# ctu-mrs/space_filling_forest_star

Measured on AMD Instinct MI355X. Metric: accepted node expansions/sec + collision checks/sec, dense_3D 6-DoF, higher is better.
Workload: dtype f64

## Files before the change

### space_filling_forest_star_amd/csrc/commit_next.h

```cpp
#pragma once
#include <stdint.h>
#include "kernels.h"
#include "sff_pmath.h"

namespace sffk {

struct CommitRegs {
  int32_t n_act, halt, n_nodes, iter, round, solved, fault, N0, iter0, n_borders, frontier_n, act_sel, act_cnt;
  int32_t app_n, app_N0, app_fn0, app_act_sel, iter0_app, app_act_cnt, app_nb0;
  unsigned long long cursor, words_base, rounds, round_nodes, round_queries, epoch;
};

SFF_HD CommitRegs commit_regs_load(const DevCtrl* c, int32_t nb0) {
  CommitRegs k{};
  k.n_act = c->n_act; k.halt = c->halt; k.iter = c->iter; k.round = c->round; k.solved = c->solved;
  k.N0 = c->N0; k.iter0 = c->iter0; k.n_borders = nb0; k.frontier_n = c->frontier_n;
  k.act_sel = c->act_sel; k.act_cnt = c->act_cnt; k.cursor = c->cursor; k.epoch = c->epoch;
  return k;
}

template <class C> SFF_HD void round_begin_next(const DevForestView& f, C* c) {
  const int cnt = c->act_cnt;
  int n = 0;
  if (c->round < f.threshold_misses && cnt > 0 && c->iter < f.max_iterations && !c->solved) {
// ... 42 lines not shown
  if (faulted) { commit_roll_back(k); return; }
  k->app_n = k->n_act;
  k->app_N0 = k->N0;
  k->app_fn0 = k->frontier_n;
  k->app_act_sel = k->act_sel;
  k->app_act_cnt = k->act_cnt;
  k->iter0_app = k->iter0;
  k->app_nb0 = k->n_borders;
  k->epoch += 1ULL;
}

template <class C> SFF_HD void commit_next_round(const DevForestView& f, C* k, int n_acc, int n_ev, bool faulted) {
  commit_applied(k, faulted);
  if (faulted) return;
  const int n = k->app_n, fn0 = k->app_fn0, act_cnt = k->app_act_cnt;
  k->n_nodes = k->app_N0 + n_acc;
  k->frontier_n = f.prio.n_heaps ? fn0 : fn0 + n_acc;
  k->n_borders = k->app_nb0 + n_ev;
  k->act_sel = k->app_act_sel ^ 1;
  k->act_cnt = (n - n_acc) + (act_cnt - n);
  round_begin_next(f, k);
}

}
```

### space_filling_forest_star_amd/csrc/devforest.hip

```cpp
#include <hip/hip_runtime.h>
#include <stdint.h>
#include <stdlib.h>
#include "kernels.h"
#include "sff_geom.h"
#include "kernels_dev.h"
#include "commit_next.h"

namespace sffk {

using namespace sffg;

__device__ __forceinline__ int record_words_dev(int nbcap) { return 6 + 4 * nbcap; }

__device__ __forceinline__ int32_t* frontier_now(const DevForestView& f) { return f.ctrl->front_sel ? f.frontier2 : f.frontier; }
__device__ __forceinline__ int32_t* act_now(const DevForestView& f) { return f.ctrl->act_sel ? f.act_slot2 : f.act_slot; }

__device__ void round_begin_scalars(const DevForestView& f, DevCtrl* c) { round_begin_next(f, c); }

#define WB_BLOCKS 64
__global__ __launch_bounds__(256) void k_wave_begin(DevForestView f) {
  __shared__ int s_last;
  __shared__ int s_scan[4];
  DevCtrl* c = f.ctrl;
  const unsigned long long tb0 = f.profile ? wall_clock64() : 0ULL;
// ... 165 lines not shown
  __syncthreads();
  if (threadIdx.x < 8) slots[threadIdx.x] = 0ULL;
  __syncthreads();
  if ((threadIdx.x & 63) == 0)
    for (int q = from; q < 8; ++q) if (v[q]) atomicAdd(&slots[q], v[q]);
  __syncthreads();
  for (int q = from; q < 8; ++q) v[q] = slots[q];
}

__device__ __forceinline__ void commit_counters(DevCtrl& K, const unsigned long long* tot, int work_items, bool have_q,
                                                unsigned long long q_beg, unsigned long long q_end) {
  K.collide_calls += tot[0];
  K.path_free_calls += tot[1];
  K.nn_queries += tot[2];
  K.poses_executed += tot[3];
  K.segments_executed += tot[4];
  K.samples_executed += tot[5];
  K.n_unsettled += (int)tot[6];
  K.work_items += (unsigned long long)work_items;
  if (have_q) { K.q_t0 = q_beg; K.q_t1 = q_end; }
  if (K.q_t1 > K.q_t0) { K.q_ticks += K.q_t1 - K.q_t0; K.q_launches += 1ULL; }
}

__global__ __launch_bounds__(1024) void k_commit(ResolveArgs A, int n_bound) {
  __shared__ int s_state[64], s_dk[64], s_dep[64];
  __shared__ unsigned long long s_cnt[64][6];
  __shared__ unsigned long long s_sum;
  __shared__ unsigned long long s_wa, s_we, s_c6[7];
  __shared__ int s_ev_total;
  __shared__ unsigned long long s_tot[8];
  __shared__ DevCtrl K;
  const DevForestView& f = A.f;
  DevCtrl* c = f.ctrl;
  const int b = blockIdx.x;
  const int grp = threadIdx.x >> 4, gl = threadIdx.x & 15, lane = threadIdx.x & 63;
  const int i = b * 64 + grp;
  const bool inb = i < n_bound;
  const size_t s0 = (size_t)i * A.stride;
  const bool inl = inb && A.in_lim[i] != 0;
  const int flags = inb ? A.rec_flags[i] : 0;
  int nnb = inb ? A.rec_nnb[i] : 0;
  const bool pose_hit = inb && A.pose_hit[i] != 0;
  int fh = 0x7fffffff, ns = 0, nb = 0, meta = 0;
  if (inb) {
    fh = A.first_hit[s0 + gl]; ns = A.seg_ns[s0 + gl];
    if (gl > 0) { nb = A.rec_nb[(size_t)i * A.nbcap + gl - 1]; meta = A.rec_meta[(size_t)i * A.nbcap + gl - 1]; }
  }
  const int halt = c->halt, n = c->n_act;
  if (halt || n == 0) {
    if (b == 0 && threadIdx.x == 0) {
      c->app_n = 0;
      if (A.star) { A.S.hdr[0] = 0; A.S.hdr[1] = 1; A.S.hdr[2] = 0; A.S.hdr[4] = 0; }
    }
    return;
  }
  if (b == 0 && f.ord.hist)
    for (int r = threadIdx.x; r < f.ord.n_sub; r += 1024) (c->act_sel ? f.ord.cnt[0] : f.ord.cnt[1])[r * SFFK_ORD_CNT_STRIDE] = 0;
  if (b * 64 >= n) return;
  const int nwg = (n + 63) >> 6;
  const bool last = b == nwg - 1;
  const unsigned seq = (unsigned)f.commit_seq[0] + 1u;
  const int seq30 = (int)(seq & 0x3fffffffu);
  const int Tb = f.temp_base, N0 = c->N0, nb0 = c->n_borders;
  const unsigned long long stamp_hi = (c->epoch + 1ULL) << 32;
  unsigned long long* pub = f.wg_pub + (size_t)b * SFFK_PUB_WORDS;
  unsigned long long tk[6];
  const bool clk = last && f.profile;
  tk[0] = clk ? wall_clock64() : 0ULL;
  unsigned long long* trace = (f.kc_trace && (int)c->rounds == f.kc_trace_round && threadIdx.x == 0) ? f.kc_trace + 8 * (size_t)b : nullptr;
#define KC_TRACE(k) do { if (trace) trace[k] = wall_clock64(); } while (0)
  KC_TRACE(0);
  const bool tail = last && A.star;
  int work_items = 0;
  if (tail) {
    for (int w = threadIdx.x; w < (int)(sizeof(DevCtrl) / 4); w += 1024)
      reinterpret_cast<int32_t*>(&K)[w] = reinterpret_cast<const int32_t*>(c)[w];
    work_items = A.round_ctrl[2];
  }
  if (!A.star && b == 0 && threadIdx.x < 64) {
    unsigned long long q_end = f.qclk_sh[threadIdx.x * 16], q_beg = f.qclk_sh[threadIdx.x * 16 + 1];
    const int wi = A.round_ctrl[2];
    for (int off = 32; off > 0; off >>= 1) {
      const unsigned long long e2 = __shfl_xor(q_end, off), b2 = __shfl_xor(q_beg, off);
      q_end = e2 > q_end ? e2 : q_end; q_beg = b2 < q_beg ? b2 : q_beg;
    }
    if (threadIdx.x == 0) {
      f.qclk_sh[KH_QBEG] = q_beg; f.qclk_sh[KH_QEND] = q_end; f.qclk_sh[KH_WORK] = (unsigned long long)wi;
      f.qclk_sh[KH_NB0] = (unsigned long long)(unsigned)nb0;
    }
  }

  auto calls_of = [](int fh, int ns) -> unsigned long long {
    return fh != 0x7fffffff ? (unsigned long long)fh : (unsigned long long)ns;
  };
  const int gsh = lane & 48;
  auto gballot = [&](bool p) -> unsigned { return (unsigned)((__ballot(p) >> gsh) & 0xffffULL); };
  auto gsum = [&](unsigned long long v) -> unsigned long long {
    for (int off = 8; off > 0; off >>= 1) v += __shfl_xor(v, off);
    return v;
  };
  unsigned long long cnt[6] = {0, 0, 0, 0, 0, 0};
  int st = 1, code = SFFK_REJECTED, dk = 0, was_dep = 0;
// ... 118 lines not shown
    const unsigned long long wa = __ballot(v == 2), we = __ballot(v == 3), wd = __ballot(s_dep[threadIdx.x] != 0);
    unsigned long long c6[6];
    for (int q = 0; q < 6; ++q) {
      c6[q] = s_cnt[threadIdx.x][q];
      for (int off = 32; off > 0; off >>= 1) c6[q] += __shfl_xor(c6[q], off);
    }
    if (threadIdx.x == 0) {
      s_wa = wa; s_we = we;
      for (int q = 0; q < 6; ++q) s_c6[q] = c6[q];
      s_c6[6] = (unsigned long long)__popcll(wd);
      f.w_acc[b] = wa;
      for (int q = 0; q < 6; ++q) kc_publish(pub + KC_CNT + q, seq, (unsigned)c6[q]);
      kc_publish(pub + KC_DEP, seq, (unsigned)__popcll(wd));
      kc_publish(pub + KC_EVN, seq, (unsigned)__popcll(we));
      kc_publish(pub + KC_WLO, seq, (unsigned)(wa & 0xffffffffULL));
      kc_publish(pub + KC_WHI, seq, (unsigned)(wa >> 32));
      kc_publish(pub + KC_ACC, seq, (unsigned)__popcll(wa));
      KC_TRACE(2);
      f.w_ev[b] = we;
    }
  }
  __syncthreads();
  const unsigned long long wa = s_wa, we = s_we;
  const bool defer = !A.star;
  int e_nb = 0, e_ex = 0, e_i = 0;
  size_t e_h = 0;
  bool is_ev = false, stamped = false, posted = false;
  if (threadIdx.x < 64) {
    if ((we >> threadIdx.x) & 1ULL) {
      is_ev = true;
      e_i = b * 64 + (int)threadIdx.x;
      const int raw = A.rec_nb[(size_t)e_i * A.nbcap + s_dk[threadIdx.x]];
      e_ex = A.parent[e_i];
      if (raw < Tb) {
        e_nb = raw;
        const int a = e_nb < e_ex ? e_nb : e_ex, bb = e_nb < e_ex ? e_ex : e_nb;
        const unsigned long long key = ((unsigned long long)(uint32_t)a << 32) | ((unsigned long long)(uint32_t)bb + 1ULL);
        e_h = border_slot(f, key);
        atomicMin(&f.bt_val[e_h], stamp_hi | (unsigned long long)(uint32_t)e_i);
        stamped = true;
        if (defer) { f.ev_h[e_i] = (unsigned long long)e_h; f.ev_nb[e_i] = e_nb; f.ev_raw[e_i] = raw; }
      }
    }
    if (!defer && __ballot(is_ev && !stamped) == 0ULL) {
      if (we != 0ULL) __threadfence();
      if (threadIdx.x == 0) {
        kc_publish(pub + KC_POSTED, seq, 1u);
        if (we == 0ULL) kc_publish(pub + KC_OWN, seq, 0u);
      }
      posted = true;
    }
  }
  unsigned long long part = 0;
  if ((int)threadIdx.x < b) part = kc_wait(f.wg_pub + (size_t)threadIdx.x * SFFK_PUB_WORDS + KC_ACC, seq, f.commit_seq + 6);
  unsigned long long early[8] = {0, 0, 0, 0, 0, 0, 0, 0};
  if (tail && (int)threadIdx.x < b)
    for (int q = 0; q < 8; ++q) early[q] = kc_load(f.wg_pub + (size_t)threadIdx.x * SFFK_PUB_WORDS + KC_CNT + q);
  const int acc_pref = (int)kc_block_sum(part, &s_sum);
  int fault_seen = 0;
  if (tail && threadIdx.x == 1023) fault_seen = __hip_atomic_load(A.fault_pending, __ATOMIC_RELAXED, __HIP_MEMORY_SCOPE_AGENT);
  if (threadIdx.x == 0) {
    f.acc_pref[b] = acc_pref;
    kc_publish(pub + KC_PREF, seq, (unsigned)acc_pref);
  }
  if (A.star && threadIdx.x < 64 && ((wa >> threadIdx.x) & 1ULL))
    A.S.acc_sample[acc_pref + __popcll(wa & ((1ULL << threadIdx.x) - 1ULL))] = b * 64 + (int)threadIdx.x;
  if (clk) tk[2] = wall_clock64();
  KC_TRACE(4);
  int n_own = 0, ev_pref = 0;
  if (f.profile && !A.star && threadIdx.x < 64) {
    const unsigned long long wm = __ballot(is_ev && !stamped);
    if (threadIdx.x == 0 && wm) atomicAdd(&f.qclk_sh[KH_MATE_EV], (unsigned long long)__popcll(wm));
  }
  if (we != 0ULL || last) {
    if (is_ev && !stamped) {
      const int raw = A.rec_nb[(size_t)e_i * A.nbcap + s_dk[threadIdx.x]];
      const int j = raw - Tb, bj = j >> 6;
      int pj = acc_pref;
      unsigned long long wj = wa;
      if (bj != b) {
        const unsigned long long* pp = f.wg_pub + (size_t)bj * SFFK_PUB_WORDS;
        pj = (int)kc_wait(pp + KC_PREF, seq, f.commit_seq + 6);
        wj = (unsigned long long)kc_wait(pp + KC_WLO, seq, f.commit_seq + 6) |
             ((unsigned long long)kc_wait(pp + KC_WHI, seq, f.commit_seq + 6) << 32);
      }
      e_nb = N0 + pj + __popcll(wj & ((1ULL << (j & 63)) - 1ULL));
      const int a = e_nb < e_ex ? e_nb : e_ex, bb = e_nb < e_ex ? e_ex : e_nb;
      const unsigned long long key = ((unsigned long long)(uint32_t)a << 32) | ((unsigned long long)(uint32_t)bb + 1ULL);
      e_h = border_slot(f, key);
      atomicMin(&f.bt_val[e_h], stamp_hi | (unsigned long long)(uint32_t)e_i);
      if (defer) { f.ev_h[e_i] = (unsigned long long)e_h; f.ev_nb[e_i] = e_nb; f.ev_raw[e_i] = raw; }
    }
  }
  if (!defer && (we != 0ULL || last)) {
    if (threadIdx.x < 64 && !posted) {
      if (we != 0ULL) __threadfence();
      if (threadIdx.x == 0) kc_publish(pub + KC_POSTED, seq, 1u);
    }
    KC_TRACE(3);
    if (we != 0ULL && (int)threadIdx.x < b) (void)kc_wait(f.wg_pub + (size_t)threadIdx.x * SFFK_PUB_WORDS + KC_POSTED, seq, f.commit_seq + 6);
    __syncthreads();
    KC_TRACE(5);
    bool own = false;
    if (is_ev) {
      const unsigned long long owner = __hip_atomic_load(&f.bt_val[e_h], __ATOMIC_RELAXED, __HIP_MEMORY_SCOPE_AGENT);
// ... 11 lines not shown
      if ((int)threadIdx.x < b) pe = kc_wait(f.wg_pub + (size_t)threadIdx.x * SFFK_PUB_WORDS + KC_OWN, seq, f.commit_seq + 6);
      ev_pref = (int)kc_block_sum(pe, &s_sum);
    }
    KC_TRACE(6);
    if (own) {
      const int at = nb0 + ev_pref + __popcll(wo & ((1ULL << threadIdx.x) - 1ULL));
      double pn[6], pe6[6], dn;
      int ta;
      const int raw = A.rec_nb[(size_t)e_i * A.nbcap + s_dk[threadIdx.x]];
      if (raw >= Tb) {
        const int j = raw - Tb;
        for (int q = 0; q < 6; ++q) pn[q] = A.newpos[6 * (size_t)j + q];
        dn = A.pdist[j] + f.d_root[A.parent[j]];
        ta = A.st.tree[A.parent[j]];
      } else {
        for (int q = 0; q < 6; ++q) pn[q] = A.st.pos[6 * (size_t)e_nb + q];
        dn = f.d_root[e_nb];
        ta = A.st.tree[e_nb];
      }
      const int tb = A.st.tree[e_ex];
      f.b_n1[at] = e_nb < e_ex ? e_nb : e_ex; f.b_n2[at] = e_nb < e_ex ? e_ex : e_nb;
      f.b_ta[at] = ta < tb ? ta : tb; f.b_tb[at] = ta < tb ? tb : ta;
      for (int q = 0; q < 6; ++q) pe6[q] = A.st.pos[6 * (size_t)e_ex + q];
      if (A.star) {
        const int e = at - nb0;
        A.S.ev_sample[e] = e_i; A.S.ev_nb[e] = e_nb; A.S.ev_ex[e] = e_ex; A.S.ev_dist[e] = dist6(pn, pe6);
        f.b_dist[at] = 0.0;
      } else
      f.b_dist[at] = dn + f.d_root[e_ex] + dist6(pn, pe6);
      f.pair[(size_t)ta * f.n_trees + tb] = 1;
      f.pair[(size_t)tb * f.n_trees + ta] = 1;
    }
  }
  KC_TRACE(7);
  if (last && !A.star && threadIdx.x == 0) {
    f.qclk_sh[KH_PASSES] = (unsigned long long)passes;
    if (clk) {
      tk[3] = wall_clock64();
      for (int q = 0; q < 3; ++q) f.qclk_sh[KH_PHASE + q] = tk[q + 1] - tk[q];
    }
  }
  if (!tail) return;
  if (clk) tk[3] = wall_clock64();
  unsigned long long q_end = 0ULL, q_beg = ~0ULL;
  if (f.qclk_sh && threadIdx.x < 64) {
    q_end = f.qclk_sh[threadIdx.x * 16]; q_beg = f.qclk_sh[threadIdx.x * 16 + 1];
    for (int off = 32; off > 0; off >>= 1) {
      const unsigned long long e2 = __shfl_xor(q_end, off), b2 = __shfl_xor(q_beg, off);
      q_end = e2 > q_end ? e2 : q_end; q_beg = b2 < q_beg ? b2 : q_beg;
    }
  }
  unsigned long long tot[8] = {0, 0, 0, 0, 0, 0, 0, 0};
  if ((int)threadIdx.x < b) {
    const unsigned long long* pp = f.wg_pub + (size_t)threadIdx.x * SFFK_PUB_WORDS;
    for (int q = 0; q < 8; ++q) tot[q] = (unsigned)(early[q] >> 32) == seq ? (unsigned)early[q] : kc_wait(pp + KC_CNT + q, seq, f.commit_seq + 6);
  }
  if (threadIdx.x == 1023) s_ev_total = fault_seen;
  kc_block_sum8(tot, s_tot, 0);
  for (int q = 0; q < 7; ++q) tot[q] += s_c6[q];
  tot[7] += (unsigned long long)__popcll(we);
  const int n_acc = acc_pref + __popcll(wa), n_ev = defer ? (int)tot[7] : ev_pref + n_own;
  const bool faulted = s_ev_total != 0;
  if (A.star && !faulted) {
    for (int w = threadIdx.x; w < (int)(sizeof(DevCtrl) / 4); w += 1024)
      reinterpret_cast<int32_t*>(A.S.backup)[w] = reinterpret_cast<const int32_t*>(&K)[w];
    __syncthreads();
    if (threadIdx.x == 0) commit_roll_back(A.S.backup);
  }
  if (threadIdx.x == 0) {
    if (faulted) {
      commit_roll_back(&K);
      *A.fault_pending = 0;
      if (A.star) { A.S.hdr[0] = 0; A.S.hdr[1] = 1; A.S.hdr[2] = 0; A.S.hdr[4] = 0; }
    } else {
      commit_counters(K, tot, work_items, f.qclk_sh != nullptr, q_beg, q_end);
      commit_next_round(f, &K, n_acc, n_ev, false);
      if (A.star) {
        K.nn_queries += (unsigned long long)n_acc;
        A.S.hdr[0] = n_acc; A.S.hdr[1] = 0; A.S.hdr[2] = n_ev; A.S.hdr[3] = nb0; A.S.hdr[4] = 0;
      }
      if (clk) {
        tk[4] = wall_clock64();
        for (int q = 0; q < 4; ++q) K.prof[q] += tk[q + 1] - tk[q];
      }
      K.prof[5] += (unsigned long long)passes;
      K.prof[6] += 1ULL;
      if ((unsigned long long)passes > K.prof[7]) K.prof[7] = (unsigned long long)passes;
    }
    f.commit_seq[0] = (int32_t)seq;
  }
  __syncthreads();
  for (int w = threadIdx.x; w < (int)(sizeof(DevCtrl) / 4); w += 1024)
    reinterpret_cast<int32_t*>(c)[w] = reinterpret_cast<const int32_t*>(&K)[w];
}

struct AppCtl {
  int32_t n, N0, fn0, act_sel, act_cnt, iter0, nb0;
  int32_t new_cnt;
  int32_t wave_over;
  int32_t ord_valid;
// ... 30 lines not shown
  h.fault = A.fault_pending[0];
  h.seq0 = f.commit_seq[0];
  return h;
}
__device__ __forceinline__ void hand_join(HandIn& h) {
  join_v(h.k.n_act, h.k.halt, h.k.iter, h.k.round, h.k.solved, h.k.N0, h.k.iter0, h.k.n_borders, h.k.frontier_n, h.k.act_sel,
         h.k.act_cnt, h.k.cursor, h.k.epoch, h.in_wave, h.use_closed, h.ord_valid, h.n_slots, h.act_identity, h.fault, h.seq0,
         h.acc, h.evn);
}
__device__ __forceinline__ bool hand_ran(const HandIn& h) { return !(h.k.halt || h.k.n_act == 0); }
__device__ __forceinline__ void hand_count_in(const ResolveArgs& A) {
  atomicAdd(&A.f.qclk_sh[(blockIdx.x & 63) * 16 + KH_READY], 1ULL);
}
__device__ __forceinline__ AppCtl hand_app_ctl(const HandIn& h, const CommitRegs& k) {
  AppCtl a{};
  a.n = k.app_n; a.N0 = k.app_N0; a.fn0 = k.app_fn0; a.act_sel = k.app_act_sel; a.act_cnt = k.app_act_cnt;
  a.iter0 = k.iter0_app; a.nb0 = k.app_nb0; a.new_cnt = k.act_cnt;
  a.wave_over = (k.n_act == 0 && !k.halt && h.in_wave && !h.use_closed) ? 1 : 0;
  a.ord_valid = h.ord_valid;
  a.seq = (unsigned)h.seq0 + 1u;
  a.epoch = k.epoch;
  return a;
}
__device__ __forceinline__ AppCtl hand_applied(const ResolveArgs& A, const HandIn& h) {
  if (!hand_ran(h)) { AppCtl a{}; a.ord_valid = h.ord_valid; return a; }
  __syncthreads();
  if (threadIdx.x == 0) hand_count_in(A);
  CommitRegs k = h.k;
  commit_applied(&k, h.fault != 0);
  return hand_app_ctl(h, k);
}
__device__ __forceinline__ AppCtl hand_derive(const ResolveArgs& A, HandIn& h, int n_lines, unsigned long long* s_part) {
  const DevForestView& f = A.f;
  if (!hand_ran(h)) { AppCtl a{}; a.ord_valid = h.ord_valid; return a; }
  const unsigned seq = (unsigned)h.seq0 + 1u;
  auto line = [&](unsigned long long acc, unsigned long long evn) -> unsigned long long {
    return ((unsigned)(acc >> 32) == seq ? (unsigned long long)(unsigned)acc : 0ULL) |
           ((unsigned)(evn >> 32) == seq ? (unsigned long long)(unsigned)evn << 32 : 0ULL);
  };
  unsigned long long v = (int)threadIdx.x < n_lines ? line(h.acc, h.evn) : 0ULL;
  for (int t = threadIdx.x + 256; t < n_lines; t += 256) {
    const unsigned long long* pp = f.wg_pub + (size_t)t * SFFK_PUB_WORDS;
    v += line(pp[KC_ACC], pp[KC_EVN]);
  }
  unsigned pk = (unsigned)v | ((unsigned)(v >> 32) << 16);
  for (int off = 32; off > 0; off >>= 1) pk += __shfl_xor(pk, off);
  if ((threadIdx.x & 63) == 0) s_part[threadIdx.x >> 6] = (unsigned long long)(pk & 0xffffu) | ((unsigned long long)(pk >> 16) << 32);
  __syncthreads();
  if (threadIdx.x == 0) hand_count_in(A);
  v = s_part[0] + s_part[1] + s_part[2] + s_part[3];
  commit_next_round(f, &h.k, (int)(unsigned)v, (int)(v >> 32), h.fault != 0);
  return hand_app_ctl(h, h.k);
}
__device__ __forceinline__ void append_ord_store(const ResolveArgs& A, const AppCtl& C, int ord_at, int next) {
  if (ord_at >= 0) (C.act_sel ? A.f.ord.lst[0] : A.f.ord.lst[1])[ord_at] = next;
}
__device__ __forceinline__ int append_one(const ResolveArgs& A, const AppCtl& C, int i, int& slot_out, int& ord_at, int part = 0) {
  ord_at = -1;
  const DevForestView& f = A.f;
  const int n = C.n;
  slot_out = -1;
  if (n <= 0) return -1;
  const int act_cnt = C.act_cnt;
  const int32_t* act_old = C.act_sel ? f.act_slot2 : f.act_slot;
  int32_t* act_new = C.act_sel ? f.act_slot : f.act_slot2;
  const bool wave_over = C.wave_over != 0;
  const bool ord_on = f.ord.hist && C.ord_valid;
  auto claim = [&](int e, int slot) {
    const int nd = f.slot_node[slot];
    atomicMin(&f.claim[nd], e);
    f.ulist[e] = nd;
  };
  if (wave_over && i == 0 && part != 1) f.ctrl->claims_done = 1;
  if (i >= n) {
    if (i < act_cnt && part != 1) {
      const int e = (C.new_cnt - (act_cnt - n)) + (i - n), slot = act_old[i];
      act_new[e] = slot;
      if (wave_over) claim(e, slot);
    }
    return -1;
  }
  const unsigned long long w = f.w_acc[i >> 6];
  const int rank = f.acc_pref[i >> 6] + __popcll(w & ((1ULL << (i & 63)) - 1ULL));
  if (!((w >> (i & 63)) & 1ULL)) {
    auto ord_append = [&](int slot) {
      const int sub = f.ord.slot_pos[slot] >> 6;
      const bool first = C.act_sel != 0;
      ord_at = sub * 64 + atomicAdd(&(first ? f.ord.cnt[0] : f.ord.cnt[1])[sub * SFFK_ORD_CNT_STRIDE], 1);
    };
    if (part == 1) {
      if (ord_on) { ord_append(act_old[i]); append_ord_store(A, C, ord_at, i - rank); }
      return -1;
    }
    slot_out = act_old[i];
    act_new[i - rank] = slot_out;
    if (ord_on && part == 0) ord_append(slot_out);
    if (wave_over) claim(i - rank, slot_out);
    return i - rank;
  }
  if (A.star) return -1;
  const int N0 = C.N0, fn0 = C.fn0;
  int32_t* const frontier = frontier_now(f);
  const int id = N0 + rank;
  const int ex = A.parent[i];
  const double* p = A.newpos + 6 * (size_t)i;
  const size_t o = (size_t)id;
// ... 142 lines not shown
    if (!faulted) {
      if (f.profile) {
        for (int q = 0; q < 3; ++q) K.prof[q] += s_stash[KH_PHASE - KH_QBEG + q];
        K.prof[3] += wall_clock64() - t0;
        K.prof[4] += s_stash[KH_MATE_EV - KH_QBEG];
      }
      K.prof[5] += passes;
      K.prof[6] += 1ULL;
      if (passes > K.prof[7]) K.prof[7] = passes;
    } else {
      *A.fault_pending = 0;
    }
    f.commit_seq[0] = (int32_t)seq;
  }
  __syncthreads();
  constexpr int W_NB = (int)(offsetof(DevCtrl, n_borders) / 4), W_CD = (int)(offsetof(DevCtrl, claims_done) / 4),
                W_Q0 = (int)(offsetof(DevCtrl, q_t0) / 4), W_Q1 = (int)(offsetof(DevCtrl, q_ticks) / 4);
  for (int w = tid; w < (int)(sizeof(DevCtrl) / 4); w += 256) {
    if (w == W_NB || w == W_CD || (sampler && w >= W_Q0 && w < W_Q1)) continue;
    reinterpret_cast<int32_t*>(c)[w] = reinterpret_cast<const int32_t*>(&K)[w];
  }
}
__global__ __launch_bounds__(256) void k_append(ResolveArgs A, int append_blocks, int n_lines) {
  __shared__ unsigned long long s_hand[4];
  if (!A.star && blockIdx.x == gridDim.x - 1) { commit_finalize(A, (int)gridDim.x - 1, false); return; }
  const bool border = (int)blockIdx.x >= append_blocks;
  AppCtl C;
  if (A.star) C = app_ctl_block(A.f);
  else if (border) {
    HandIn h = hand_request<false>(A, n_lines);
    hand_join(h);
    C = hand_applied(A, h);
  } else {
    HandIn h = hand_request<true>(A, n_lines);
    hand_join(h);
    C = hand_derive(A, h, n_lines, s_hand);
  }
  if (border) { border_finalize(A, C, (int)blockIdx.x - append_blocks); return; }
  int slot, ord_at;
  const int next = append_one(A, C, blockIdx.x * 256 + threadIdx.x, slot, ord_at);
  append_ord_store(A, C, ord_at, next);
}
struct ListOne { int i, n, act_cnt, app_sel, new_cnt, slot, ex, next; bool wave_over; };
__device__ __forceinline__ void append_list_request(const ResolveArgs& A, int i, int bound, int n_lines, HandIn& h, SampleCtl& K,
                                                    ListOne& L) {
  const DevForestView& f = A.f;
  const DevCtrl* c = f.ctrl;
  const int ic = i < bound ? i : bound - 1;
  if (!A.star) h = hand_request<true>(A, n_lines);
  unsigned long long w = f.w_acc[ic >> 6];
  int pref = f.acc_pref[ic >> 6];
  int s0 = f.act_slot[ic], s1 = f.act_slot2[ic];
  int ex = A.parent[ic];
  L.i = i; L.n = 0; L.act_cnt = 0; L.app_sel = 0; L.new_cnt = 0; L.wave_over = false;
  if (A.star) {
    K = sample_ctl(c);
    int n = c->app_n, act_cnt = c->app_act_cnt, app_sel = c->app_act_sel, new_cnt = c->act_cnt;
    int in_wave = c->in_wave, use_closed = c->use_closed;
    join_ctl_v(K);
    join_v(n, act_cnt, app_sel, new_cnt, in_wave, use_closed, w, pref, s0, s1, ex);
    L.n = n; L.act_cnt = act_cnt; L.app_sel = app_sel; L.new_cnt = new_cnt;
    L.wave_over = K.n == 0 && !K.halt && in_wave && !use_closed;
  } else {
    hand_join(h);
    join_v(w, pref, s0, s1, ex);
    K = SampleCtl{};
    K.words_base = h.k.cursor;
    if (hand_ran(h)) {
      CommitRegs k = h.k;
      commit_applied(&k, h.fault != 0);
      L.n = k.app_n; L.act_cnt = k.app_act_cnt; L.app_sel = k.app_act_sel;
    }
  }
  L.slot = L.app_sel ? s1 : s0;
  L.ex = ex;
  L.next = (i < L.n && !((w >> (i & 63)) & 1ULL)) ? i - (pref + __popcll(w & ((1ULL << (i & 63)) - 1ULL))) : -1;
}
__device__ __forceinline__ void append_list_store(const ResolveArgs& A, const ListOne& L) {
  const DevForestView& f = A.f;
  const int i = L.i, n = L.n;
  if (n <= 0) return;
  int32_t* act_new = L.app_sel ? f.act_slot : f.act_slot2;
  if (L.wave_over && i == 0) f.ctrl->claims_done = 1;
  if (i >= n) {
    if (i < L.act_cnt) {
      const int e = (L.new_cnt - (L.act_cnt - n)) + (i - n);
      act_new[e] = L.slot;
      if (L.wave_over) { const int nd = f.slot_node[L.slot]; atomicMin(&f.claim[nd], e); f.ulist[e] = nd; }
    }
    return;
  }
  if (L.next < 0) return;
  act_new[L.next] = L.slot;
  if (L.wave_over) { atomicMin(&f.claim[L.ex], L.next); f.ulist[L.next] = L.ex; }
}
__global__ __launch_bounds__(256) void k_append_sample(ResolveArgs A, SampleLaunch P, int append_blocks, int n_lines) {
  __shared__ unsigned long long s_hand[4];
  if (!A.star && blockIdx.x == gridDim.x - 1) { commit_finalize(A, (int)gridDim.x - 1, true); return; }
  const int nb = append_blocks;
  const bool sampler = (int)blockIdx.x >= nb && (int)blockIdx.x < 2 * nb;
  if (!sampler) {
    AppCtl C;
    if (A.star) C = app_ctl_block(A.f);
    else {
      HandIn h = hand_request<false>(A, n_lines);
      hand_join(h);
      C = hand_applied(A, h);
    }
    if ((int)blockIdx.x >= 2 * nb) { border_finalize(A, C, (int)blockIdx.x - 2 * nb); return; }
    int slot, ord_at;
    (void)append_one(A, C, blockIdx.x * 256 + threadIdx.x, slot, ord_at, 1);
    return;
  }
  const int tid = ((int)blockIdx.x - nb) * 256 + threadIdx.x;
  HandIn h{};
  SampleCtl K;
  ListOne L;
  append_list_request(A, tid, P.n, n_lines, h, K, L);
  if (!A.star) {
    const AppCtl C = hand_derive(A, h, n_lines, s_hand);
    K.n = h.k.n_act; K.halt = h.k.halt; K.act_sel = h.k.act_sel; K.round = h.k.round;
    K.ord_valid = h.ord_valid; K.n_slots = h.n_slots; K.act_identity = h.act_identity;
    L.new_cnt = C.new_cnt; L.wave_over = C.wave_over != 0;
  }
  append_list_store(A, L);
  if (K.halt) return;
  const bool valid = L.next >= 0 && L.next < K.n;
  const SampleIn S = sample_fetch(valid ? L.next : 0, valid ? L.ex : 0, K, P);
  sample_finish(tid, valid, L.next, valid ? L.ex : 0, S, -1, K, P);
}

__device__ void wave_end_control(const DevForestView& f, DevCtrl* c, int removed, int fn, bool from_closed, int n_fail,
                                 const int32_t* grid_ovf, const int32_t* tgrid_ovf, const unsigned long long* star_s) {
  c->closed_n += removed;
  if (f.prio.n_heaps) {
    c->compact_from = 0;
    c->empty_frontier = c->prio_all_empty;
  } else {
    c->compact_from = removed > 0 ? fn : 0;
    c->frontier_n = fn - removed;
    if (removed > 0) c->front_sel ^= 1;
    c->empty_frontier = c->frontier_n == 0 ? 1 : 0;
  }
  if (!c->solved && c->empty_frontier && f.goal_id < 0) {
    const int R = f.n_trees;
    int reached = 1;
    for (int t = 0; t < R; ++t) f.claim[t] = t == 0 ? 1 : 0;
// ... 219 lines not shown
  else if (k < 4 + 2 * A.nbcap) A.rec_meta[(size_t)i * A.nbcap + (k - 4 - A.nbcap)] = v;
  else if (k < 4 + 2 * A.nbcap + A.stride) A.seg_ns[s0 + (k - 4 - 2 * A.nbcap)] = v;
  else A.first_hit[s0 + (k - 4 - 2 * A.nbcap - A.stride)] = v;
}

__global__ __launch_bounds__(256) void k_border_rehash(DevForestView f, int n) {
  const int e = blockIdx.x * 256 + threadIdx.x;
  if (e >= n) return;
  const unsigned long long key = ((unsigned long long)(uint32_t)f.b_n1[e] << 32) | ((unsigned long long)(uint32_t)f.b_n2[e] + 1ULL);
  const size_t h = border_slot(f, key);
  f.bt_val[h] = 0ULL;
}

void launch_wave_begin_only(hipStream_t s, const DevForestView& f);
void launch_wave_begin(hipStream_t s, const DevForestView& f) {
  launch_wave_begin_only(s, f);
  if (f.prio.n_heaps) launch_prio_begin(s, f);
}
void launch_wave_begin_only(hipStream_t s, const DevForestView& f) {
  hipLaunchKernelGGL(k_wave_begin, dim3(WB_BLOCKS), dim3(256), 0, s, f);
}
void launch_commit(hipStream_t s, const ResolveArgs& a, int n_bound, const StarLaunch* star, const SampleLaunch* next) {
  if (n_bound <= 0) return;
  hipLaunchKernelGGL(k_commit, dim3((n_bound + 63) / 64), dim3(1024), 0, s, a, n_bound);
  if (a.star && star) launch_star_stage(s, a, n_bound, *star);
  const int ab = (n_bound + 255) / 256, lines = (n_bound + 63) / 64, fb = a.star ? 0 : lines + 1;
  if (next) hipLaunchKernelGGL(k_append_sample, dim3(2 * ab + fb), dim3(256), 0, s, a, *next, ab, lines);
  else hipLaunchKernelGGL(k_append, dim3(ab + fb), dim3(256), 0, s, a, ab, lines);
}
void launch_wave_end(hipStream_t s, const DevForestView& f, const int32_t* grid_ovf, const int32_t* tgrid_ovf,
                     unsigned long long* star_acc) {
  hipLaunchKernelGGL(k_wave_end_wide, dim3((f.wave + 255) / 256), dim3(256), 0, s, f, grid_ovf, tgrid_ovf, star_acc);
  hipLaunchKernelGGL(k_frontier_compact, dim3(512), dim3(256), 0, s, f);
}
void launch_pack_records(hipStream_t s, const ResolveArgs& a, int rank, int world, int n_bound, int32_t* send) {
  const int per_rank = (n_bound + world - 1) / world;
  const long long threads = (long long)per_rank * record_words(a.nbcap);
  hipLaunchKernelGGL(k_pack_records, dim3((unsigned)((threads + 255) / 256)), dim3(256), 0, s, a, rank, world, send);
}
void launch_unpack_records(hipStream_t s, const ResolveArgs& a, int rank, int world, int n_bound, const int32_t* recv) {
  const int per_rank = (n_bound + world - 1) / world;
  const long long threads = (long long)n_bound * record_words(a.nbcap);
  hipLaunchKernelGGL(k_unpack_records, dim3((unsigned)((threads + 255) / 256)), dim3(256), 0, s, a, rank, world, per_rank, recv);
}
void launch_border_rehash(hipStream_t s, const DevForestView& f, int n) {
  if (n <= 0) return;
  hipLaunchKernelGGL(k_border_rehash, dim3((n + 255) / 256), dim3(256), 0, s, f, n);
// ... 4 lines not shown
```

### space_filling_forest_star_amd/csrc/forest_dev.cpp

```cpp
#include <algorithm>
#include <chrono>
#include <cmath>
#include <cstdio>
#include <cstdlib>
#include <cstring>
#include <thread>
#include <vector>

#include "engine.h"
#include "sff_geom.h"

namespace sff {

#define HIPCHK(x) hip_check((x), #x)
using Clock = std::chrono::steady_clock;
static double ms_since(Clock::time_point t0) { return std::chrono::duration<double, std::milli>(Clock::now() - t0).count(); }

static uint64_t next_pow2(uint64_t v) {
  uint64_t p = 1;
  while (p < v) p <<= 1;
  return p;
}

bool Forest::device_eligible() const {
// ... 1583 lines not shown
      }
    }
    const double r = (double)std::max<unsigned long long>(1ULL, k.prof[6]);
    if (d.kc_trace.p) {
      const size_t nw = (size_t)cfg.wave / 64 + 2;
      std::vector<unsigned long long> tr(nw * 8);
      HIPCHK(hipMemcpy(tr.data(), d.kc_trace.p, nw * 64, hipMemcpyDeviceToHost));
      unsigned long long t0 = ~0ULL;
      size_t used = 0;
      for (size_t w = 0; w < nw; ++w) if (tr[8 * w]) { t0 = std::min(t0, tr[8 * w]); used = w + 1; }
      static const char* names[8] = {"start", "walk done", "count published", "stamps posted", "lower counts in (ids)", "lower stamps in", "lower owned counts in", "end"};
      for (int k = 0; k < 8 && used; ++k) {
        std::vector<double> v;
        for (size_t w = 0; w < used; ++w) if (tr[8 * w + k]) v.push_back((double)(tr[8 * w + k] - t0) / 100.0);
        if (v.empty()) continue;
        std::vector<double> sv = v;
        std::sort(sv.begin(), sv.end());
        fprintf(stderr, "[sffgpu k_commit trace, %zu workgroups] %-24s us after the first start: min %.1f median %.1f max %.1f | first wg %.1f last wg %.1f\n",
                used, names[k], sv.front(), sv[sv.size() / 2], sv.back(), v.front(), v.back());
      }
    }
    fprintf(stderr, "[sffgpu k_commit us/commit, last workgroup] walks + waits for earlier samples %.1f (%.2f polls, max %llu) "
            "lower workgroups' counts %.1f borders %.1f | control block (%s) %.1f | dependent/round %.0f | "
            "border events with a neighbour accepted in the same round %llu\n", k.prof[0] / r / 100.0, k.prof[5] / r,
            (unsigned long long)k.prof[7], k.prof[1] / r / 100.0, k.prof[2] / r / 100.0,
            cfg.optimize ? "in k_commit" : "finalize block of the append launch", k.prof[3] / r / 100.0,
            (double)k.n_unsettled / r, (unsigned long long)k.prof[4]);
#ifdef SFFK_CI_TRACE
    {
      std::vector<unsigned long long> tr(4096 * 8);
      sffk::debug_ci_trace(tr.data());
      unsigned long long t0 = ~0ULL, tend = 0;
      for (int w = 0; w < 4096; ++w) if (tr[8 * w]) { t0 = std::min(t0, tr[8 * w]); tend = std::max(tend, tr[8 * w + 7]); }
      struct It { double start, broad, end; int nc, smp, items, wave; double entry, pre; };
      std::vector<It> its;
      int waves = 0, n_pose_items = 0;
      double pose_us = 0, pose_max = 0;
      for (int w = 0; w < 4096; ++w) {
        if (!tr[8 * w]) continue;
        ++waves;
        { const unsigned long long pp = tr[8 * w + 6] >> 8; n_pose_items += (int)(pp & 0xff); pose_us += (double)(pp >> 8) / 100.0; if ((pp & 0xff) && (double)(pp >> 8) / 100.0 > pose_max) pose_max = (double)(pp >> 8) / 100.0; tr[8 * w + 6] &= 0xff; }
        if (!tr[8 * w + 6]) continue;
        its.push_back({(tr[8 * w + 1] - t0) / 100.0, tr[8 * w + 2] >= tr[8 * w + 1] ? (tr[8 * w + 2] - t0) / 100.0 : -1.0, (tr[8 * w + 3] - t0) / 100.0,
                       (int)tr[8 * w + 4], (int)(tr[8 * w + 5] & 0xff), (int)tr[8 * w + 6], w, (tr[8 * w] - t0) / 100.0, ((tr[8 * w + 5] >> 8) - t0) / 100.0});
      }
      std::sort(its.begin(), its.end(), [](const It& a, const It& b) { return a.end > b.end; });
      fprintf(stderr, "[sffgpu k_collide_items trace] %d waves, %zu with items, kernel %.1f us (first start -> last end)\n", waves, its.size(), (tend - t0) / 100.0);
      for (size_t k = 0; k < its.size() && k < 12; ++k)
        fprintf(stderr, "  wave %4d: entry %.1f preamble done %.1f | items %d | first item: start %.1f broad done %.1f end %.1f us | candidates %d masked samples %d\n",
                its[k].wave, its[k].entry, its[k].pre, its[k].items, its[k].start, its[k].broad, its[k].end, its[k].nc, its[k].smp);
// ... 42 lines not shown
```

Baseline: 11.65 million.

## Drop cross-workgroup accepted-prefix chain from non-star commit; recompute prefixes in append

Templates k_commit on STAR. In the non-star path, a workgroup no longer waits on every lower workgroup's published accept count to build its prefix. It waits only when it has border events whose neighbour is still unstamped, and then sums just the lower groups' counts for that mate's group. The append kernels rebuild the per-line accepted prefixes locally from the published words using a DPP wave scan in shared memory, instead of reading f.acc_pref. This cuts the serial decoupled-lookback chain in k_commit, at the cost of redundant scans in every append block and more code complexity.

```diff
diff --git a/space_filling_forest_star_amd/csrc/commit_next.h b/space_filling_forest_star_amd/csrc/commit_next.h
--- a/space_filling_forest_star_amd/csrc/commit_next.h
+++ b/space_filling_forest_star_amd/csrc/commit_next.h
@@ -88,4 +88,31 @@
   round_begin_next(f, k);
 }
 
+SFF_HD unsigned commit_line_count(unsigned long long word, unsigned seq) {
+  return (unsigned)(word >> 32) == seq ? (unsigned)word : 0u;
 }
+#define SFFK_LINE_CHUNKS (SFFK_DEV_MAX_GROUPS / 64)
+SFF_HD int commit_prefix_base(const unsigned long long* part, int g) {
+  const int c = g >> 6;
+  const int p0 = (int)(unsigned)part[0], p1 = (int)(unsigned)part[1], p2 = (int)(unsigned)part[2], p3 = (int)(unsigned)part[3];
+  int base = (c > 0 ? p0 : 0) + (c > 1 ? p1 : 0) + (c > 2 ? p2 : 0) + (c > 3 ? p3 : 0);
+  for (int k = 4; k < c; ++k) base += (int)(unsigned)part[k];
+  return base;
+}
+SFF_HD int commit_line_prefix(const unsigned long long* acc, int stride, int n_lines, unsigned seq, int32_t* pref) {
+  if (n_lines < 0 || n_lines > SFFK_DEV_MAX_GROUPS) return -1;
+  unsigned long long part[SFFK_LINE_CHUNKS] = {};
+  const int chunks = (n_lines + 63) >> 6;
+  for (int k = 0; k < chunks; ++k) {
+    unsigned run = 0;
+    for (int g = k * 64; g < n_lines && g < k * 64 + 64; ++g) {
+      pref[g] = (int32_t)run;
+      run += commit_line_count(acc[(size_t)g * (size_t)stride], seq);
+    }
+    part[k] = run;
+  }
+  for (int g = 0; g < n_lines; ++g) pref[g] += commit_prefix_base(part, g);
+  return commit_prefix_base(part, chunks * 64);
+}
+
+}
diff --git a/space_filling_forest_star_amd/csrc/devforest.hip b/space_filling_forest_star_amd/csrc/devforest.hip
--- a/space_filling_forest_star_amd/csrc/devforest.hip
+++ b/space_filling_forest_star_amd/csrc/devforest.hip
@@ -211,13 +211,15 @@
   if (K.q_t1 > K.q_t0) { K.q_ticks += K.q_t1 - K.q_t0; K.q_launches += 1ULL; }
 }
 
-__global__ __launch_bounds__(1024) void k_commit(ResolveArgs A, int n_bound) {
+template <bool STAR> __global__ __launch_bounds__(1024) void k_commit(ResolveArgs A, int n_bound) {
   __shared__ int s_state[64], s_dk[64], s_dep[64];
   __shared__ unsigned long long s_cnt[64][6];
   __shared__ unsigned long long s_sum;
   __shared__ unsigned long long s_wa, s_we, s_c6[7];
   __shared__ int s_ev_total;
   __shared__ unsigned long long s_tot[8];
+  __shared__ unsigned long long s_wm;
+  __shared__ int s_bj[64];
   __shared__ DevCtrl K;
   const DevForestView& f = A.f;
   DevCtrl* c = f.ctrl;
@@ -239,7 +241,7 @@
   if (halt || n == 0) {
     if (b == 0 && threadIdx.x == 0) {
       c->app_n = 0;
-      if (A.star) { A.S.hdr[0] = 0; A.S.hdr[1] = 1; A.S.hdr[2] = 0; A.S.hdr[4] = 0; }
+      if (STAR) { A.S.hdr[0] = 0; A.S.hdr[1] = 1; A.S.hdr[2] = 0; A.S.hdr[4] = 0; }
     }
     return;
   }
@@ -259,14 +261,14 @@
   unsigned long long* trace = (f.kc_trace && (int)c->rounds == f.kc_trace_round && threadIdx.x == 0) ? f.kc_trace + 8 * (size_t)b : nullptr;
 #define KC_TRACE(k) do { if (trace) trace[k] = wall_clock64(); } while (0)
   KC_TRACE(0);
-  const bool tail = last && A.star;
+  const bool tail = last && STAR;
   int work_items = 0;
   if (tail) {
     for (int w = threadIdx.x; w < (int)(sizeof(DevCtrl) / 4); w += 1024)
       reinterpret_cast<int32_t*>(&K)[w] = reinterpret_cast<const int32_t*>(c)[w];
     work_items = A.round_ctrl[2];
   }
-  if (!A.star && b == 0 && threadIdx.x < 64) {
+  if (!STAR && b == 0 && threadIdx.x < 64) {
     unsigned long long q_end = f.qclk_sh[threadIdx.x * 16], q_beg = f.qclk_sh[threadIdx.x * 16 + 1];
     const int wi = A.round_ctrl[2];
     for (int off = 32; off > 0; off >>= 1) {
@@ -431,7 +433,7 @@
   }
   __syncthreads();
   const unsigned long long wa = s_wa, we = s_we;
-  const bool defer = !A.star;
+  const bool defer = STAR ? !A.star : true;
   int e_nb = 0, e_ex = 0, e_i = 0;
   size_t e_h = 0;
   bool is_ev = false, stamped = false, posted = false;
@@ -460,36 +462,62 @@
       posted = true;
     }
   }
-  unsigned long long part = 0;
-  if ((int)threadIdx.x < b) part = kc_wait(f.wg_pub + (size_t)threadIdx.x * SFFK_PUB_WORDS + KC_ACC, seq, f.commit_seq + 6);
+  int acc_pref = 0;
   unsigned long long early[8] = {0, 0, 0, 0, 0, 0, 0, 0};
-  if (tail && (int)threadIdx.x < b)
-    for (int q = 0; q < 8; ++q) early[q] = kc_load(f.wg_pub + (size_t)threadIdx.x * SFFK_PUB_WORDS + KC_CNT + q);
-  const int acc_pref = (int)kc_block_sum(part, &s_sum);
   int fault_seen = 0;
-  if (tail && threadIdx.x == 1023) fault_seen = __hip_atomic_load(A.fault_pending, __ATOMIC_RELAXED, __HIP_MEMORY_SCOPE_AGENT);
-  if (threadIdx.x == 0) {
-    f.acc_pref[b] = acc_pref;
-    kc_publish(pub + KC_PREF, seq, (unsigned)acc_pref);
-  }
-  if (A.star && threadIdx.x < 64 && ((wa >> threadIdx.x) & 1ULL))
-    A.S.acc_sample[acc_pref + __popcll(wa & ((1ULL << threadIdx.x) - 1ULL))] = b * 64 + (int)threadIdx.x;
+  if constexpr (STAR) {
+    unsigned long long part = 0;
+    if ((int)threadIdx.x < b) part = kc_wait(f.wg_pub + (size_t)threadIdx.x * SFFK_PUB_WORDS + KC_ACC, seq, f.commit_seq + 6);
+    if (tail && (int)threadIdx.x < b)
+      for (int q = 0; q < 8; ++q) early[q] = kc_load(f.wg_pub + (size_t)threadIdx.x * SFFK_PUB_WORDS + KC_CNT + q);
+    acc_pref = (int)kc_block_sum(part, &s_sum);
+    if (tail && threadIdx.x == 1023) fault_seen = __hip_atomic_load(A.fault_pending, __ATOMIC_RELAXED, __HIP_MEMORY_SCOPE_AGENT);
+    if (threadIdx.x == 0) {
+      f.acc_pref[b] = acc_pref;
+      kc_publish(pub + KC_PREF, seq, (unsigned)acc_pref);
+    }
+    if (threadIdx.x < 64 && ((wa >> threadIdx.x) & 1ULL))
+      A.S.acc_sample[acc_pref + __popcll(wa & ((1ULL << threadIdx.x) - 1ULL))] = b * 64 + (int)threadIdx.x;
+  }
   if (clk) tk[2] = wall_clock64();
   KC_TRACE(4);
   int n_own = 0, ev_pref = 0;
-  if (f.profile && !A.star && threadIdx.x < 64) {
-    const unsigned long long wm = __ballot(is_ev && !stamped);
-    if (threadIdx.x == 0 && wm) atomicAdd(&f.qclk_sh[KH_MATE_EV], (unsigned long long)__popcll(wm));
-  }
-  if (we != 0ULL || last) {
+  int mate_pref = acc_pref;
+  if constexpr (!STAR) {
+    if (we != 0ULL) {
+      if (threadIdx.x < 64) {
+        const bool m = is_ev && !stamped;
+        int bj = b;
+        if (m) bj = (A.rec_nb[(size_t)e_i * A.nbcap + s_dk[threadIdx.x]] - Tb) >> 6;
+        const unsigned long long wm = __ballot(m), wx = __ballot(m && bj != b);
+        s_bj[threadIdx.x] = bj;
+        if (threadIdx.x == 0) {
+          s_wm = wm;
+          if (f.profile && wm) atomicAdd(&f.qclk_sh[KH_MATE_EV], (unsigned long long)__popcll(wm) | ((unsigned long long)__popcll(wx) << 32));
+        }
+      }
+      __syncthreads();
+      const unsigned long long wm = s_wm;
+      if (wm != 0ULL) {
+        unsigned long long part = 0;
+        if ((int)threadIdx.x < b) part = kc_wait(f.wg_pub + (size_t)threadIdx.x * SFFK_PUB_WORDS + KC_ACC, seq, f.commit_seq + 6);
+        for (unsigned long long m = wm; m; m &= m - 1ULL) {
+          const int e = __ffsll((long long)m) - 1;
+          const int below = (int)kc_block_sum((int)threadIdx.x < s_bj[e] ? part : 0ULL, &s_sum);
+          if ((int)threadIdx.x == e) mate_pref = below;
+        }
+      }
+    }
+  }
+  if (we != 0ULL || (STAR && last)) {
     if (is_ev && !stamped) {
       const int raw = A.rec_nb[(size_t)e_i * A.nbcap + s_dk[threadIdx.x]];
       const int j = raw - Tb, bj = j >> 6;
-      int pj = acc_pref;
+      int pj = mate_pref;
       unsigned long long wj = wa;
       if (bj != b) {
         const unsigned long long* pp = f.wg_pub + (size_t)bj * SFFK_PUB_WORDS;
-        pj = (int)kc_wait(pp + KC_PREF, seq, f.commit_seq + 6);
+        if constexpr (STAR) pj = (int)kc_wait(pp + KC_PREF, seq, f.commit_seq + 6);
         wj = (unsigned long long)kc_wait(pp + KC_WLO, seq, f.commit_seq + 6) |
              ((unsigned long long)kc_wait(pp + KC_WHI, seq, f.commit_seq + 6) << 32);
       }
@@ -547,7 +575,7 @@
       f.b_n1[at] = e_nb < e_ex ? e_nb : e_ex; f.b_n2[at] = e_nb < e_ex ? e_ex : e_nb;
       f.b_ta[at] = ta < tb ? ta : tb; f.b_tb[at] = ta < tb ? tb : ta;
       for (int q = 0; q < 6; ++q) pe6[q] = A.st.pos[6 * (size_t)e_ex + q];
-      if (A.star) {
+      if (STAR) {
         const int e = at - nb0;
         A.S.ev_sample[e] = e_i; A.S.ev_nb[e] = e_nb; A.S.ev_ex[e] = e_ex; A.S.ev_dist[e] = dist6(pn, pe6);
         f.b_dist[at] = 0.0;
@@ -558,7 +586,7 @@
     }
   }
   KC_TRACE(7);
-  if (last && !A.star && threadIdx.x == 0) {
+  if (last && !STAR && threadIdx.x == 0) {
     f.qclk_sh[KH_PASSES] = (unsigned long long)passes;
     if (clk) {
       tk[3] = wall_clock64();
@@ -586,7 +614,7 @@
   tot[7] += (unsigned long long)__popcll(we);
   const int n_acc = acc_pref + __popcll(wa), n_ev = defer ? (int)tot[7] : ev_pref + n_own;
   const bool faulted = s_ev_total != 0;
-  if (A.star && !faulted) {
+  if (STAR && !faulted) {
     for (int w = threadIdx.x; w < (int)(sizeof(DevCtrl) / 4); w += 1024)
       reinterpret_cast<int32_t*>(A.S.backup)[w] = reinterpret_cast<const int32_t*>(&K)[w];
     __syncthreads();
@@ -596,11 +624,11 @@
     if (faulted) {
       commit_roll_back(&K);
       *A.fault_pending = 0;
-      if (A.star) { A.S.hdr[0] = 0; A.S.hdr[1] = 1; A.S.hdr[2] = 0; A.S.hdr[4] = 0; }
+      if (STAR) { A.S.hdr[0] = 0; A.S.hdr[1] = 1; A.S.hdr[2] = 0; A.S.hdr[4] = 0; }
     } else {
       commit_counters(K, tot, work_items, f.qclk_sh != nullptr, q_beg, q_end);
       commit_next_round(f, &K, n_acc, n_ev, false);
-      if (A.star) {
+      if (STAR) {
         K.nn_queries += (unsigned long long)n_acc;
         A.S.hdr[0] = n_acc; A.S.hdr[1] = 0; A.S.hdr[2] = n_ev; A.S.hdr[3] = nb0; A.S.hdr[4] = 0;
       }
@@ -677,40 +705,66 @@
   a.epoch = k.epoch;
   return a;
 }
-__device__ __forceinline__ AppCtl hand_applied(const ResolveArgs& A, const HandIn& h) {
+__device__ __forceinline__ AppCtl hand_applied(const ResolveArgs& A, const HandIn& h, bool counted_in = false) {
   if (!hand_ran(h)) { AppCtl a{}; a.ord_valid = h.ord_valid; return a; }
-  __syncthreads();
-  if (threadIdx.x == 0) hand_count_in(A);
+  if (!counted_in) {
+    __syncthreads();
+    if (threadIdx.x == 0) hand_count_in(A);
+  }
   CommitRegs k = h.k;
   commit_applied(&k, h.fault != 0);
   return hand_app_ctl(h, k);
 }
-__device__ __forceinline__ AppCtl hand_derive(const ResolveArgs& A, HandIn& h, int n_lines, unsigned long long* s_part) {
+struct HandLds {
+  unsigned long long part[SFFK_LINE_CHUNKS];
+  int pref[4];
+};
+__device__ __forceinline__ unsigned wave_scan_add(unsigned v) {
+  int x = (int)v;
+  x += __builtin_amdgcn_update_dpp(0, x, 0x111, 0xf, 0xf, false);
+  x += __builtin_amdgcn_update_dpp(0, x, 0x112, 0xf, 0xf, false);
+  x += __builtin_amdgcn_update_dpp(0, x, 0x114, 0xf, 0xf, false);
+  x += __builtin_amdgcn_update_dpp(0, x, 0x118, 0xf, 0xf, false);
+  x += __builtin_amdgcn_update_dpp(0, x, 0x142, 0xa, 0xf, false);
+  x += __builtin_amdgcn_update_dpp(0, x, 0x143, 0xc, 0xf, false);
+  return (unsigned)x;
+}
+__device__ __forceinline__ int hand_chunks(int n_lines) {
+  const int k = (n_lines + 63) >> 6;
+  return k < SFFK_LINE_CHUNKS ? k : SFFK_LINE_CHUNKS;
+}
+__device__ __forceinline__ void hand_lines(const ResolveArgs& A, const HandIn& h, int n_lines, int g0, HandLds* s) {
   const DevForestView& f = A.f;
+  const unsigned seq = (unsigned)h.seq0 + 1u;
+  const int lane = threadIdx.x & 63;
+  unsigned long long acc = h.acc, evn = h.evn;
+  for (int l = threadIdx.x; l < 256 || l < 64 * hand_chunks(n_lines); l += 256) {
+    if (l >= 256) {
+      const unsigned long long* pp = f.wg_pub + (size_t)(l < n_lines ? l : 0) * SFFK_PUB_WORDS;
+      acc = pp[KC_ACC]; evn = pp[KC_EVN];
+    }
+    const unsigned pk = l < n_lines ? commit_line_count(acc, seq) | (commit_line_count(evn, seq) << 16) : 0u;
+    const unsigned inc = wave_scan_add(pk);
+    if ((unsigned)(l - g0) < 4u) s->pref[l - g0] = (int)((inc - pk) & 0xffffu);
+    if (lane == 63) s->part[l >> 6] = (unsigned long long)(inc & 0xffffu) | ((unsigned long long)(inc >> 16) << 32);
+  }
+  __syncthreads();
+  if (threadIdx.x == 0) hand_count_in(A);
+}
+__device__ __forceinline__ int hand_prefix(const HandLds* s, int g) { return commit_prefix_base(s->part, g) + s->pref[g & 3]; }
+__device__ __forceinline__ AppCtl hand_derive(const ResolveArgs& A, HandIn& h, int n_lines, int g0, HandLds* s) {
   if (!hand_ran(h)) { AppCtl a{}; a.ord_valid = h.ord_valid; return a; }
-  const unsigned seq = (unsigned)h.seq0 + 1u;
-  auto line = [&](unsigned long long acc, unsigned long long evn) -> unsigned long long {
-    return ((unsigned)(acc >> 32) == seq ? (unsigned long long)(unsigned)acc : 0ULL) |
-           ((unsigned)(evn >> 32) == seq ? (unsigned long long)(unsigned)evn << 32 : 0ULL);
-  };
-  unsigned long long v = (int)threadIdx.x < n_lines ? line(h.acc, h.evn) : 0ULL;
-  for (int t = threadIdx.x + 256; t < n_lines; t += 256) {
-    const unsigned long long* pp = f.wg_pub + (size_t)t * SFFK_PUB_WORDS;
-    v += line(pp[KC_ACC], pp[KC_EVN]);
-  }
-  unsigned pk = (unsigned)v | ((unsigned)(v >> 32) << 16);
-  for (int off = 32; off > 0; off >>= 1) pk += __shfl_xor(pk, off);
-  if ((threadIdx.x & 63) == 0) s_part[threadIdx.x >> 6] = (unsigned long long)(pk & 0xffffu) | ((unsigned long long)(pk >> 16) << 32);
-  __syncthreads();
-  if (threadIdx.x == 0) hand_count_in(A);
-  v = s_part[0] + s_part[1] + s_part[2] + s_part[3];
-  commit_next_round(f, &h.k, (int)(unsigned)v, (int)(v >> 32), h.fault != 0);
+  hand_lines(A, h, n_lines, g0, s);
+  unsigned long long v = s->part[0] + s->part[1] + s->part[2] + s->part[3];
+  for (int k = 4; k < hand_chunks(n_lines); ++k) v += s->part[k];
+  commit_next_round(A.f, &h.k, (int)(unsigned)v, (int)(v >> 32), h.fault != 0);
   return hand_app_ctl(h, h.k);
 }
 __device__ __forceinline__ void append_ord_store(const ResolveArgs& A, const AppCtl& C, int ord_at, int next) {
   if (ord_at >= 0) (C.act_sel ? A.f.ord.lst[0] : A.f.ord.lst[1])[ord_at] = next;
 }
-__device__ __forceinline__ int append_one(const ResolveArgs& A, const AppCtl& C, int i, int& slot_out, int& ord_at, int part = 0) {
+__device__ __forceinline__ int append_one(const ResolveArgs& A, const AppCtl& C, const HandLds* hs, int i, int& slot_out, int& ord_at,
+                                          int part = 0) {
   ord_at = -1;
   const DevForestView& f = A.f;
   const int n = C.n;
@@ -736,7 +790,7 @@
     return -1;
   }
   const unsigned long long w = f.w_acc[i >> 6];
-  const int rank = f.acc_pref[i >> 6] + __popcll(w & ((1ULL << (i & 63)) - 1ULL));
+  const int rank = (hs ? hand_prefix(hs, i >> 6) : f.acc_pref[i >> 6]) + __popcll(w & ((1ULL << (i & 63)) - 1ULL));
   if (!((w >> (i & 63)) & 1ULL)) {
     auto ord_append = [&](int slot) {
       const int sub = f.ord.slot_pos[slot] >> 6;
@@ -925,7 +979,7 @@
   }
 }
 __global__ __launch_bounds__(256) void k_append(ResolveArgs A, int append_blocks, int n_lines) {
-  __shared__ unsigned long long s_hand[4];
+  __shared__ HandLds s_hand;
   if (!A.star && blockIdx.x == gridDim.x - 1) { commit_finalize(A, (int)gridDim.x - 1, false); return; }
   const bool border = (int)blockIdx.x >= append_blocks;
   AppCtl C;
@@ -937,14 +991,14 @@
   } else {
     HandIn h = hand_request<true>(A, n_lines);
     hand_join(h);
-    C = hand_derive(A, h, n_lines, s_hand);
+    C = hand_derive(A, h, n_lines, 4 * (int)blockIdx.x, &s_hand);
   }
   if (border) { border_finalize(A, C, (int)blockIdx.x - append_blocks); return; }
   int slot, ord_at;
-  const int next = append_one(A, C, blockIdx.x * 256 + threadIdx.x, slot, ord_at);
+  const int next = append_one(A, C, A.star ? nullptr : &s_hand, blockIdx.x * 256 + threadIdx.x, slot, ord_at);
   append_ord_store(A, C, ord_at, next);
 }
-struct ListOne { int i, n, act_cnt, app_sel, new_cnt, slot, ex, next; bool wave_over; };
+struct ListOne { int i, n, act_cnt, app_sel, new_cnt, slot, ex, next, pref; unsigned long long w; bool wave_over; };
 __device__ __forceinline__ void append_list_request(const ResolveArgs& A, int i, int bound, int n_lines, HandIn& h, SampleCtl& K,
                                                     ListOne& L) {
   const DevForestView& f = A.f;
@@ -952,7 +1006,7 @@
   const int ic = i < bound ? i : bound - 1;
   if (!A.star) h = hand_request<true>(A, n_lines);
   unsigned long long w = f.w_acc[ic >> 6];
-  int pref = f.acc_pref[ic >> 6];
+  int pref = A.star ? f.acc_pref[ic >> 6] : 0;
   int s0 = f.act_slot[ic], s1 = f.act_slot2[ic];
   int ex = A.parent[ic];
   L.i = i; L.n = 0; L.act_cnt = 0; L.app_sel = 0; L.new_cnt = 0; L.wave_over = false;
@@ -966,7 +1020,7 @@
     L.wave_over = K.n == 0 && !K.halt && in_wave && !use_closed;
   } else {
     hand_join(h);
-    join_v(w, pref, s0, s1, ex);
+    join_v(w, s0, s1, ex);
     K = SampleCtl{};
     K.words_base = h.k.cursor;
     if (hand_ran(h)) {
@@ -977,7 +1031,11 @@
   }
   L.slot = L.app_sel ? s1 : s0;
   L.ex = ex;
-  L.next = (i < L.n && !((w >> (i & 63)) & 1ULL)) ? i - (pref + __popcll(w & ((1ULL << (i & 63)) - 1ULL))) : -1;
+  L.w = w; L.pref = pref; L.next = -1;
+}
+__device__ __forceinline__ void append_list_next(ListOne& L) {
+  const int i = L.i;
+  L.next = (i < L.n && !((L.w >> (i & 63)) & 1ULL)) ? i - (L.pref + __popcll(L.w & ((1ULL << (i & 63)) - 1ULL))) : -1;
 }
 __device__ __forceinline__ void append_list_store(const ResolveArgs& A, const ListOne& L) {
   const DevForestView& f = A.f;
@@ -998,21 +1056,27 @@
   if (L.wave_over) { atomicMin(&f.claim[L.ex], L.next); f.ulist[L.next] = L.ex; }
 }
 __global__ __launch_bounds__(256) void k_append_sample(ResolveArgs A, SampleLaunch P, int append_blocks, int n_lines) {
-  __shared__ unsigned long long s_hand[4];
+  __shared__ HandLds s_hand;
   if (!A.star && blockIdx.x == gridDim.x - 1) { commit_finalize(A, (int)gridDim.x - 1, true); return; }
   const int nb = append_blocks;
   const bool sampler = (int)blockIdx.x >= nb && (int)blockIdx.x < 2 * nb;
   if (!sampler) {
+    const bool border = (int)blockIdx.x >= 2 * nb;
     AppCtl C;
     if (A.star) C = app_ctl_block(A.f);
-    else {
+    else if (border) {
       HandIn h = hand_request<false>(A, n_lines);
       hand_join(h);
       C = hand_applied(A, h);
-    }
-    if ((int)blockIdx.x >= 2 * nb) { border_finalize(A, C, (int)blockIdx.x - 2 * nb); return; }
+    } else {
+      HandIn h = hand_request<true>(A, n_lines);
+      hand_join(h);
+      if (hand_ran(h)) hand_lines(A, h, n_lines, 4 * (int)blockIdx.x, &s_hand);
+      C = hand_applied(A, h, true);
+    }
+    if (border) { border_finalize(A, C, (int)blockIdx.x - 2 * nb); return; }
     int slot, ord_at;
-    (void)append_one(A, C, blockIdx.x * 256 + threadIdx.x, slot, ord_at, 1);
+    (void)append_one(A, C, A.star ? nullptr : &s_hand, blockIdx.x * 256 + threadIdx.x, slot, ord_at, 1);
     return;
   }
   const int tid = ((int)blockIdx.x - nb) * 256 + threadIdx.x;
@@ -1021,11 +1085,13 @@
   ListOne L;
   append_list_request(A, tid, P.n, n_lines, h, K, L);
   if (!A.star) {
-    const AppCtl C = hand_derive(A, h, n_lines, s_hand);
+    const AppCtl C = hand_derive(A, h, n_lines, 4 * ((int)blockIdx.x - nb), &s_hand);
+    if (tid < L.n) L.pref = hand_prefix(&s_hand, tid >> 6);
     K.n = h.k.n_act; K.halt = h.k.halt; K.act_sel = h.k.act_sel; K.round = h.k.round;
     K.ord_valid = h.ord_valid; K.n_slots = h.n_slots; K.act_identity = h.act_identity;
     L.new_cnt = C.new_cnt; L.wave_over = C.wave_over != 0;
   }
+  append_list_next(L);
   append_list_store(A, L);
   if (K.halt) return;
   const bool valid = L.next >= 0 && L.next < K.n;
@@ -1291,7 +1357,8 @@
 }
 void launch_commit(hipStream_t s, const ResolveArgs& a, int n_bound, const StarLaunch* star, const SampleLaunch* next) {
   if (n_bound <= 0) return;
-  hipLaunchKernelGGL(k_commit, dim3((n_bound + 63) / 64), dim3(1024), 0, s, a, n_bound);
+  if (a.star) hipLaunchKernelGGL(k_commit<true>, dim3((n_bound + 63) / 64), dim3(1024), 0, s, a, n_bound);
+  else hipLaunchKernelGGL(k_commit<false>, dim3((n_bound + 63) / 64), dim3(1024), 0, s, a, n_bound);
   if (a.star && star) launch_star_stage(s, a, n_bound, *star);
   const int ab = (n_bound + 255) / 256, lines = (n_bound + 63) / 64, fb = a.star ? 0 : lines + 1;
   if (next) hipLaunchKernelGGL(k_append_sample, dim3(2 * ab + fb), dim3(256), 0, s, a, *next, ab, lines);
diff --git a/space_filling_forest_star_amd/csrc/forest_dev.cpp b/space_filling_forest_star_amd/csrc/forest_dev.cpp
--- a/space_filling_forest_star_amd/csrc/forest_dev.cpp
+++ b/space_filling_forest_star_amd/csrc/forest_dev.cpp
@@ -1629,10 +1629,10 @@
     }
     fprintf(stderr, "[sffgpu k_commit us/commit, last workgroup] walks + waits for earlier samples %.1f (%.2f polls, max %llu) "
             "lower workgroups' counts %.1f borders %.1f | control block (%s) %.1f | dependent/round %.0f | "
-            "border events with a neighbour accepted in the same round %llu\n", k.prof[0] / r / 100.0, k.prof[5] / r,
+            "border events with a neighbour accepted in the same round %llu, in a lower workgroup %llu\n", k.prof[0] / r / 100.0, k.prof[5] / r,
             (unsigned long long)k.prof[7], k.prof[1] / r / 100.0, k.prof[2] / r / 100.0,
             cfg.optimize ? "in k_commit" : "finalize block of the append launch", k.prof[3] / r / 100.0,
-            (double)k.n_unsettled / r, (unsigned long long)k.prof[4]);
+            (double)k.n_unsettled / r, (unsigned long long)(k.prof[4] & 0xffffffffULL), (unsigned long long)(k.prof[4] >> 32));
 #ifdef SFFK_CI_TRACE
     {
       std::vector<unsigned long long> tr(4096 * 8);
```

New measurement: 12.00 million, median of 6. 1.03x the previous value.
